# yannickBurkhardt/LongTermPlanner

Measured on AMD Instinct MI355X. Metric: 7-DoF trajectory plans/sec (batch 1M), higher is better.
Workload: dtype f64; 1 GPU; 1000000 x 7-DoF queries per GPU per step, limits 'panda', Tsample 0.001 s, full q/v/a/j sampling into a reused 192.0 GiB tile (2 chunks per step); batch_per_gpu=1000000, global_batch=1000000, dof=7, workload_key=panda:1000000:f64, limits=panda, input_layout=query_major, table_pass=auto, batches_in_flight=1, semantics=cpp, pow_rule=libm, backend=none (single rank), plans_ok_is=planTrajectory's bool

## Files before the change

### longtermplanner_amd/csrc/ltp_device.hpp

```cpp
#pragma once
#include "ltp_kernels.hpp"
#include "ltp_profile.hpp"

namespace ltp {

typedef double double2_t __attribute__((ext_vector_type(2)));
typedef float float4_t __attribute__((ext_vector_type(4)));

template <typename T> struct OutVec;
template <> struct OutVec<double> { typedef double2_t type; static constexpr int N = 2; };
template <> struct OutVec<float> { typedef float4_t type; static constexpr int N = 4; };

LTP_DEV LimPow load_limit_powers(const Limits& lim, int j)
{
    const double* w = lim.pw + (long long)j * kLimPowN;
    return LimPow{w[0], w[1], w[2], w[3], w[4], w[5], w[6]};
}

LTP_DEV JointLimits load_limits(const Limits& lim, int j)
{
    JointLimits L;
    L.q_min = lim.q_min[j];
    L.q_max = lim.q_max[j];
    L.v_max = lim.v_max[j];
    L.a_max = lim.a_max[j];
    L.j_max = lim.j_max[j];
    L.pw = load_limit_powers(lim, j);
    return L;
}

LTP_DEV int plan_set(const PlanLimits& lim, long long p)
{
    const int s = lim.set_index[p];
    return s >= 0 && s < lim.n_sets ? s : -1;
}

LTP_DEV Limits plan_limits(const PlanLimits& lim, long long p, int dof)
{
    if (!lim.set_index) return lim;
    const int s = plan_set(lim, p);
    const long long o = (long long)(s < 0 ? 0 : s) * dof, rows = lim.set_rows;
    return Limits{lim.sets + o, lim.sets + rows + o, lim.sets + 2 * rows + o, lim.sets + 3 * rows + o, lim.sets + 4 * rows + o,
                  lim.set_pw + o * kLimPowN};
}

struct PlanLane {
    bool live;
    long long local, p;
    int j;
    LTP_DEV void start(const Queries& in, double& q, double& v, double& a) const
    {
        const long long ix = p * in.sq + (long long)j * in.sj;
        q = in.q_0[ix];
        v = in.v_0[ix];
        a = in.a_0[ix];
    }
};
LTP_DEV PlanLane plan_lane(const PlanRange& r)
{
    const long long idx = (long long)blockIdx.x * blockDim.x + threadIdx.x;
    const long long local = idx / r.dof;
    return PlanLane{idx < r.count * r.dof, local, r.first + local, (int)(idx - local * r.dof)};
}

LTP_DEV bool beyond_end_limits(double q, double q_min, double q_max) { return q < q_min || q > q_max; }

LTP_DEV int joint_len(const double (&t)[7], double t_sample)
{
    bool finite = true;
#pragma unroll
    for (int k = 0; k < 7; ++k) finite = finite && dfinite(t[k]);
    const double len = dceil(t[6] / t_sample) + 1.0;
    return (finite && len < 2147483647.0) ? (int)len : -1;
}

LTP_HD int stored_len(int len, RowSpec rows)
{
    if (len <= 0) return 0;
    const int st = rows.stride > 1 ? rows.stride : 1;
    const int cnt = (len + st - 1) / st;
    return (rows.max_samples > 0 && cnt > rows.max_samples) ? rows.max_samples : cnt;
}

LTP_DEV unsigned long long plan_size(int len, int dof)
{
    if (len <= 0) return 0ull;
    const unsigned long long stride = ((unsigned long long)len + (kRowAlign - 1)) / kRowAlign * kRowAlign;
    return 4ull * (unsigned long long)dof * stride;
}

}
```

### longtermplanner_amd/csrc/ltp_sampler.hip

```cpp
#include "ltp_sampler_lds.hpp"

namespace ltp {

template <bool STREAMING, bool DRY, typename T>
__global__ void __launch_bounds__(kSampleThreads, (sizeof(T) == 4 ? kSampleBlocksPerCU - 1 : kSampleBlocksPerCU))
k_sample(long long first, long long count, int dof, double t_sample, PlanLimits lim, Queries in, Records rec,
         const unsigned long long* __restrict__ offsets, T* __restrict__ out, unsigned long long capacity,
         unsigned long long* __restrict__ stamps, int spread, RowSpec rows, unsigned long long* __restrict__ next_item,
         int draw_chunk )
{
    __shared__ SegTable tab;
    __shared__ unsigned long long s_item;
    const int ngroups = (dof + kSampleJointGroup - 1) / kSampleJointGroup;
    const long long per = (count + spread - 1) / spread;
    const unsigned long long total = (unsigned long long)per * spread * ngroups;
    const unsigned long long off0 = offsets[first];
    unsigned long long chunk_base = 0ull;
    int chunk_i = 0;
    auto draw = [&]() -> unsigned long long {
        if (chunk_i == 0) chunk_base = atomicAdd(next_item, (unsigned long long)draw_chunk);
        return chunk_base + (unsigned long long)chunk_i;
    };

    auto decode = [&](unsigned long long item, long long& local, int& j0, int& nj) {
        const int group = (int)(item % ngroups);
        const long long slot = (long long)(item / ngroups);
        local = (slot % spread) * per + slot / spread;
        j0 = group * kSampleJointGroup;
        nj = (dof - j0) < kSampleJointGroup ? (dof - j0) : kSampleJointGroup;
    };
    auto fetch = [&](unsigned long long item) {
        long long local; int j0, nj;
        decode(item, local, j0, nj);
        const bool some = item < total && local < count;
        return fetch_item<false>(some ? first + local : -1, j0, nj, dof, lim, in, rec, offsets);
    };

    if (threadIdx.x == 0) s_item = draw();
    chunk_i = (chunk_i + 1) & (draw_chunk - 1);
    __syncthreads();
    unsigned long long item = s_item;
    ItemRegs<false> cur = fetch(item);
    __syncthreads();
    while (item < total) {
        long long local; int j0, nj;
        decode(item, local, j0, nj);
        const long long p = first + local;
        const bool lead = threadIdx.x == 0 && j0 == 0;
        if (stamps && lead && local < count) stamps[3 * local] = wall_clock64();
        const int len = __builtin_amdgcn_readfirstlane(cur.len);
        const unsigned long long off = ((unsigned long long)(unsigned)__builtin_amdgcn_readfirstlane((int)(unsigned)(cur.off >> 32)) << 32) |
                                       (unsigned long long)(unsigned)__builtin_amdgcn_readfirstlane((int)(unsigned)cur.off);
        const unsigned long long rel = off - off0;
        const int slen = stored_len(len, rows);
        const unsigned long long stride = ((unsigned long long)slen + (kRowAlign - 1)) / kRowAlign * kRowAlign;
        bool ok = len > 0;
        if (ok && rel + 4ull * dof * stride > capacity) {
            if (lead) atomicOr(&rec.status[p], kStatusOverflow);
            ok = false;
        }
        unsigned long long drawn = 0ull;
        if (threadIdx.x == 0) drawn = draw();
        chunk_i = (chunk_i + 1) & (draw_chunk - 1);
        if (ok) build_run_tables(tab, p, j0, nj, len, t_sample, plan_limits(lim, p, dof), rec, cur.pa, cur.pb);
        if (threadIdx.x == 0) s_item = drawn;
        __syncthreads();
        const unsigned long long nitem = s_item;
        const ItemRegs<false> nxt = fetch(nitem);
        if (ok) {
            if (stamps && lead) stamps[3 * local + 1] = wall_clock64();
            stream_rows<STREAMING, DRY, T>(tab, j0, nj, dof, slen, stride, out + rel, rows);
        }
        __syncthreads();
        if (stamps && ok && lead) stamps[3 * local + 2] = wall_clock64();
        item = nitem;
        cur = nxt;
    }
}

int sample_resident_blocks(int device, bool f32)
{
    int cus = 0, per_cu = 0;
    if (hipDeviceGetAttribute(&cus, hipDeviceAttributeMultiprocessorCount, device) != hipSuccess || cus <= 0) cus = 256;
    hipError_t e;
    if (f32) e = hipOccupancyMaxActiveBlocksPerMultiprocessor(&per_cu, k_sample<true, false, float>, kSampleThreads, 0);
    else e = hipOccupancyMaxActiveBlocksPerMultiprocessor(&per_cu, k_sample<true, false, double>, kSampleThreads, 0);
    if (e != hipSuccess || per_cu <= 0) per_cu = 4;
    return cus * per_cu;
}

void launch_sample(hipStream_t s, const PlanRange& r, const unsigned long long* offsets, void* out, bool f32, unsigned long long capacity,
                   bool nontemporal, bool dry, int interleave, RowSpec rows, unsigned long long* next_item, int resident_blocks,
                   unsigned long long* stamps)
{
    const long long count = r.count;
    const int dof = r.dof;
    if (count <= 0) return;
    int spread = interleave != 0 ? interleave : kSampleSpread;
    if ((long long)spread > count) spread = (int)count;
    const int ngroups = (dof + kSampleJointGroup - 1) / kSampleJointGroup;
    long long blocks = resident_blocks > 0 ? resident_blocks : 1536;
    if (blocks > count * ngroups) blocks = count * ngroups;
    const dim3 grid((unsigned)blocks);
    const dim3 block(kSampleThreads);
    const int draw_chunk = queue_draw_chunk(rows, f32, dof < kSampleJointGroup ? dof : kSampleJointGroup);
#define LTP_SAMPLE_CASE(ST, DR, TY) hipLaunchKernelGGL((k_sample<ST, DR, TY>), grid, block, 0, s, r.first, count, dof, r.t_sample, r.lim, r.in, r.rec, offsets, (TY*)out, capacity, stamps, spread, rows, next_item, draw_chunk)
    switch ((nontemporal ? 1 : 0) | (dry ? 2 : 0) | (f32 ? 4 : 0)) {
    case 0: LTP_SAMPLE_CASE(false, false, double); break;
    case 1: LTP_SAMPLE_CASE(true, false, double); break;
    case 2: LTP_SAMPLE_CASE(false, true, double); break;
    case 3: LTP_SAMPLE_CASE(true, true, double); break;
    case 4: LTP_SAMPLE_CASE(false, false, float); break;
    case 5: LTP_SAMPLE_CASE(true, false, float); break;
    case 6: LTP_SAMPLE_CASE(false, true, float); break;
    default: LTP_SAMPLE_CASE(true, true, float); break;
    }
#undef LTP_SAMPLE_CASE
}

}
```

### longtermplanner_amd/csrc/ltp_sampler_lds.hpp

```cpp
#pragma once
#include "ltp_runs.hpp"

namespace ltp {

struct SegScratch {
    int s[kSampleJointGroup][8];
    double fr[kSampleJointGroup][8];
    double frts[kSampleJointGroup][8];
    double misc[kSampleJointGroup][8];
    double Jp[kSampleJointGroup][8];
    double corr[kSampleJointGroup][10];
    int cand[kSampleJointGroup][kMaxSegments];
    double runJ[kSampleJointGroup][kMaxSegments];
    int runMode[kSampleJointGroup][kMaxSegments];
    double state[kSampleJointGroup][kMaxSegments][3];
};
struct SegTable {
    JointTable jt[kSampleJointGroup];
    union {
        SegScratch w;
        double2_t bnd[kSampleJointGroup][kMaxSegments][4];
    };
};
static_assert(kSampleJointGroup == kRunTableJoints && kSampleThreads == kRunTableThreads, "install_run_tables is written for this block shape");

constexpr int kCutSlots = 20;
__device__ const signed char kCutBase[kCutSlots] = {0, 0, 0, 0, 1, 1, 2, 2, 2, 3, 3, 3, 4, 4, 4, 5, 5, 6, 6, 6};
__device__ const signed char kCutDelta[kCutSlots] = {0, 0, 1, 2, 0, 1, 0, 1, 2, -1, 0, 1, 0, 1, 2, 0, 1, 0, 1, 2};

LTP_DEV void wave_sync()
{
    __builtin_amdgcn_fence(__ATOMIC_RELEASE, "wavefront");
    __builtin_amdgcn_wave_barrier();
    __builtin_amdgcn_fence(__ATOMIC_ACQUIRE, "wavefront");
}

template <bool TABLES>
struct ItemRegs {
    int len;
    unsigned long long off;
    double pa, pb;
    unsigned long long w[kTableLoads];
};
template <>
struct ItemRegs<false> {
    int len;
    unsigned long long off;
    double pa, pb;
};

template <bool TABLES>
LTP_DEV ItemRegs<TABLES> fetch_item(long long p, int j0, int nj, int dof, const PlanLimits& lim, const Queries& in, const Records& rec,
                                    const unsigned long long* __restrict__ offsets,
                                    const unsigned long long* __restrict__ tables = nullptr, long long tab_first = 0)
{
    ItemRegs<TABLES> r;
    r.len = 0; r.off = 0ull; r.pa = 0.0; r.pb = 0.0;
    if constexpr (TABLES) {
#pragma unroll
        for (int x = 0; x < kTableLoads; ++x) r.w[x] = 0ull;
    }
    if (p < 0) return r;
    r.len = rec.traj_len[p];
    if (offsets) r.off = offsets[p];
    if constexpr (TABLES) {
        const PackedTableRegs t = fetch_run_tables(tables, (unsigned long long)(p - tab_first) * dof + j0, nj);
#pragma unroll
        for (int x = 0; x < kTableLoads; ++x) r.w[x] = t.w[x];
        return r;
    }
    const int jl = threadIdx.x >> 5, k = threadIdx.x & 31;
    if (jl < nj) {
        const int j = j0 + jl;
        const long long rj = p * dof + j;
        const long long ix = p * in.sq + (long long)j * in.sj;
        if (k < 7) r.pa = rec.t_scaled[rj * 7 + k];
        else if (k == 7) { r.pa = rec.dir[rj]; r.pb = plan_limits(lim, p, dof).j_max[j]; }
        else if (k == 8) { r.pa = rec.v_drive[rj]; r.pb = rec.dir[rj]; }
        else if (k == 9) r.pa = in.q_0[ix];
        else if (k == 10) r.pa = in.v_0[ix];
        else if (k == 11) r.pa = in.a_0[ix];
        else if (k == 12) r.pa = (double)rec.mod[rj];
    }
    return r;
}

template <bool PROBE = false>
LTP_DEV void build_run_tables(SegTable& tab, long long p, int j0, int nj, int len, double Ts, const Limits& lim,
                              const Records& rec, double pa, double pb, unsigned long long* probe = nullptr)
{
    __builtin_amdgcn_s_setprio(3);
    const int jl = threadIdx.x >> 5, k = threadIdx.x & 31;
    const bool jact = jl < nj;
    const int j = j0 + (jact ? jl : 0);
    if (jact && k < 7) {
        const double tk = pa;
        const double fr = tk - Ts * dfloor(tk / Ts);
        tab.w.fr[jl][k] = fr;
        tab.w.frts[jl][k] = fr / Ts;
        tab.w.s[jl][k] = (k & 1) ? (int)dceil(tk / Ts) : (int)dfloor(tk / Ts);
    } else if (jact && k < 13) {
        tab.w.misc[jl][k - 7] = k < 9 ? pa * pb : pa;
    }
    wave_sync();
    if constexpr (PROBE) { if (threadIdx.x == 0) probe[3] = wall_clock64(); }
    int cval = -1;
    if (jact && k == 8) {
        const double dj = tab.w.misc[jl][0];
        const bool modp = tab.w.misc[jl][5] == 1.0;
        const double J0 = dj * (modp ? -1.0 : 1.0), J2 = dj * (modp ? 1.0 : -1.0), J4 = dj * -1.0, J6 = dj * 1.0;
        tab.w.Jp[jl][0] = J0; tab.w.Jp[jl][1] = dj * 0.0; tab.w.Jp[jl][2] = J2; tab.w.Jp[jl][3] = dj * 0.0;
        tab.w.Jp[jl][4] = J4; tab.w.Jp[jl][5] = dj * 0.0; tab.w.Jp[jl][6] = J6;
        const double* ft = tab.w.frts[jl];
        const double d20 = (tab.w.fr[jl][2] - tab.w.fr[jl][0]) / Ts;
        tab.w.corr[jl][0] = ft[0] * J0;
        tab.w.corr[jl][1] = (1 - ft[1]) * J2;
        tab.w.corr[jl][2] = ft[2] * J2;
        tab.w.corr[jl][3] = d20 * J2;
        tab.w.corr[jl][4] = (1 - ft[3]) * J4;
        tab.w.corr[jl][5] = ft[4] * J4;
        tab.w.corr[jl][6] = 0.0;
        tab.w.corr[jl][7] = (1 - ft[5]) * J6;
        tab.w.corr[jl][8] = ft[6] * J6;
    }
    if (jact && k < kCutSlots) {
        const int c = k == 0 ? 0 : tab.w.s[jl][kCutBase[k]] + kCutDelta[k];
        cval = (k == 0 || (c > 0 && c < len)) ? c : -1;
        tab.w.cand[jl][k] = cval;
    }
    wave_sync();
    if constexpr (PROBE) { if (threadIdx.x == 0) probe[4] = wall_clock64(); }
    if (jact && k < kCutSlots) {
        bool first = cval >= 0;
#pragma unroll
        for (int m = 0; m < kCutSlots; ++m) first = first && (m >= k || tab.w.cand[jl][m] != cval);
        tab.w.runMode[jl][k] = first ? cval : -1;
    }
    wave_sync();
    if constexpr (PROBE) { if (threadIdx.x == 0) probe[5] = wall_clock64(); }
    if (jact && k < kCutSlots) {
        const bool mine = tab.w.runMode[jl][k] >= 0;
        int pos = 0, distinct = 0;
#pragma unroll
        for (int m = 0; m < kCutSlots; ++m) {
            const int cm = tab.w.runMode[jl][m];
            if (cm >= 0) { ++distinct; if (cm < cval) ++pos; }
        }
        if (mine) tab.jt[jl].start[pos] = cval;
        if (k == 0) { tab.jt[jl].start[distinct] = len; tab.jt[jl].nseg = distinct; }
    }
    wave_sync();
    if constexpr (PROBE) { if (threadIdx.x == 0) probe[6] = wall_clock64(); }
    const int ns = jact ? tab.jt[jl].nseg : 0;
    if (k < ns) {
        const int b = tab.jt[jl].start[k];
        const int* sj = tab.w.s[jl];
        const bool phase4 = sj[3] - sj[2] > 2;
        int mode = 0;
        if (b > sj[6]) mode |= kModeTail;
        if (phase4 && b >= sj[2] + 1 && b < sj[3] - 1) mode |= kModeVSnap;
        const double J = jerk_at(sj, tab.w.Jp[jl], tab.w.corr[jl], b);
        tab.w.runMode[jl][k] = mode;
        tab.w.runJ[jl][k] = J;
        reinterpret_cast<int*>(tab.jt[jl].c[k])[0] = tab.jt[jl].start[k + 1] - b;
    }
    wave_sync();
    if constexpr (PROBE) { if (threadIdx.x == 0) probe[7] = wall_clock64(); }
    if (jact && k == 0) {
        const double vsnap = tab.w.misc[jl][1];
        double q = tab.w.misc[jl][2], v = tab.w.misc[jl][3], a = tab.w.misc[jl][4];
        int mode = tab.w.runMode[jl][0], cnt = reinterpret_cast<const int*>(tab.jt[jl].c[0])[0];
        double J = tab.w.runJ[jl][0];
        for (int m = 0; m < ns; ++m) {
            const int mn = m + 1 < ns ? m + 1 : m;
            const int mode_n = tab.w.runMode[jl][mn], cnt_n = reinterpret_cast<const int*>(tab.jt[jl].c[mn])[0];
            const double J_n = tab.w.runJ[jl][mn];
            tab.w.state[jl][m][0] = a; tab.w.state[jl][m][1] = v; tab.w.state[jl][m][2] = q;
            const RunCoef rc = run_coef(mode, J, a, v, q, vsnap, Ts);
            double jj;
            run_eval(rc.c, cnt, q, v, a, jj);
            mode = mode_n; cnt = cnt_n; J = J_n;
        }
        if (beyond_end_limits(q, lim.q_min[j], lim.q_max[j])) atomicOr(&rec.status[p], kStatusEndLimit);
    }
    wave_sync();
    if constexpr (PROBE) { if (threadIdx.x == 0) probe[8] = wall_clock64(); }
    if (k < ns) {
        const RunCoef rc = run_coef(tab.w.runMode[jl][k], tab.w.runJ[jl][k], tab.w.state[jl][k][0], tab.w.state[jl][k][1],
                                    tab.w.state[jl][k][2], tab.w.misc[jl][1], Ts);
#pragma unroll
        for (int x = 0; x < kRunCoefs; ++x) tab.jt[jl].c[k][x] = rc.c[x];
    }
    __builtin_amdgcn_s_setprio(0);
}

template <bool STREAMING, bool DRY, typename T>
LTP_DEV void stream_rows(SegTable& tab, int j0, int nj, int dof, int slen, unsigned long long stride, T* __restrict__ plan_base,
                         RowSpec rows)
{
    typedef typename OutVec<T>::type V;
    constexpr int N = OutVec<T>::N;
    const unsigned long long arr_stride = (unsigned long long)dof * stride;
    const int nslots = (slen + N - 1) / N;
    const int sstride = rows.stride > 1 ? rows.stride : 1;

    if constexpr (!DRY) {
        const int jl = threadIdx.x >> 5, k = threadIdx.x & 31;
        const int nruns = jl < nj ? tab.jt[jl].nseg : 0;
        if (k < nruns) {
            const int* st = tab.jt[jl].start;
            const int u = k >= 1 ? (st[k] + sstride - 1) / sstride
                                 : slen;
            bool mine = (u % N) != 0 && u < N * nslots;
            if (mine && k > 1) {
                const int up = (st[k - 1] + sstride - 1) / sstride;
                if ((up % N) != 0 && up / N == u / N) mine = false;
            }
            if (mine) {
                const int i0 = u / N * N, t0 = i0 * sstride;
                int kh = k >= 1 ? k - 1 : nruns - 1;
                while (st[kh] > t0) --kh;
                int ch = st[kh], nh = kh + 1 < nruns ? st[kh + 1] : 0x7fffffff;
                V o[4];
#pragma unroll
                for (int h = 0; h < N; ++h) {
                    const int i = t0 + h * sstride;
                    while (nh <= i) {
                        ++kh;
                        ch = nh;
                        nh = kh + 1 < nruns ? st[kh + 1] : 0x7fffffff;
                    }
                    const bool pad = i0 + h >= slen;
                    double x4[4];
                    run_eval(tab.jt[jl].c[kh], i - ch + 1, x4[0], x4[1], x4[2], x4[3]);
#pragma unroll
                    for (int x = 0; x < 4; ++x) o[x][h] = pad ? (T)0 : (T)x4[x];
                }
#pragma unroll
                for (int x = 0; x < 4; ++x) *reinterpret_cast<V*>(&tab.bnd[jl][k][x]) = o[x];
            }
        }
        __syncthreads();
    }

    const int lw = nslots <= 64 ? 0 : (nslots <= 128 ? 1 : 2);
    const int wave = __builtin_amdgcn_readfirstlane((int)(threadIdx.x >> 6)), lane = threadIdx.x & 63;
    typedef unsigned int u32x4 __attribute__((ext_vector_type(4)));
    constexpr int kWindowSlots = 1 << 26;
    constexpr bool kBufferStores = STREAMING && sizeof(T) == 8;
    for (int jl2 = wave >> lw; jl2 < nj; jl2 += 4 >> lw) {
        T* const row = plan_base + (unsigned long long)(j0 + jl2) * stride;
        const int* st = tab.jt[jl2].start;
        const int nruns = tab.jt[jl2].nseg;
        int kr = 0, cur = 0, nxt = nruns > 1 ? st[1] : 0x7fffffff;
        for (int wbase = 0; wbase < nslots; wbase += kWindowSlots) {
            const int wend = nslots - wbase < kWindowSlots ? nslots : wbase + kWindowSlots;
            __amdgpu_buffer_rsrc_t rsrc[4];
            if constexpr (kBufferStores) {
#pragma unroll
                for (int x = 0; x < 4; ++x) {
                    rsrc[x] = __builtin_amdgcn_make_buffer_rsrc(row + x * arr_stride + (unsigned long long)wbase * N, 0,
                                                                (wend - wbase) * (int)sizeof(V), 0x00020000);
                }
            }
            for (int slot = wbase + ((wave & ((1 << lw) - 1)) << 6) + lane; slot < wend; slot += 64 << lw) {
                const int i0 = N * slot;
                V o[4];
                if constexpr (DRY) {
#pragma unroll
                    for (int x = 0; x < 4; ++x)
#pragma unroll
                        for (int h = 0; h < N; ++h) o[x][h] = (T)(i0 + h);
                } else {
                    const int t0 = i0 * sstride;
                    while (nxt <= t0) {
                        ++kr;
                        cur = nxt;
                        nxt = kr + 1 < nruns ? st[kr + 1] : 0x7fffffff;
                    }
                    const bool straddles = t0 + (N - 1) * sstride >= nxt;
                    if (straddles || i0 + N > slen) {
                        const int e = straddles ? kr + 1 : 0;
#pragma unroll
                        for (int x = 0; x < 4; ++x) o[x] = *reinterpret_cast<const V*>(&tab.bnd[jl2][e][x]);
                    } else {
                        double c[kRunCoefs];
#pragma unroll
                        for (int x = 0; x < kRunCoefs; ++x) c[x] = tab.jt[jl2].c[kr][x];
#pragma unroll
                        for (int h = 0; h < N; ++h) {
                            double x4[4];
                            run_eval(c, t0 + h * sstride - cur + 1, x4[0], x4[1], x4[2], x4[3]);
#pragma unroll
                            for (int x = 0; x < 4; ++x) o[x][h] = (T)x4[x];
                        }
                    }
                }
                if constexpr (kBufferStores) {
                    const unsigned voff = (unsigned)(slot - wbase) * (unsigned)sizeof(V);
#pragma unroll
                    for (int x = 0; x < 4; ++x)
                        __builtin_amdgcn_raw_buffer_store_b128(__builtin_bit_cast(u32x4, o[x]), rsrc[x], voff, 0,  2 | 16);
                } else if constexpr (STREAMING) {
#pragma unroll
                    for (int x = 0; x < 4; ++x) __builtin_nontemporal_store(o[x], reinterpret_cast<V*>(row + x * arr_stride + i0));
                } else {
#pragma unroll
                    for (int x = 0; x < 4; ++x) *reinterpret_cast<V*>(row + x * arr_stride + i0) = o[x];
                }
            }
        }
    }
}

}
```

Baseline: 17.86 million plans/s.

## Prefetch next item's plan words via scalar loads and deepen work-draw pipeline

The sampler kernel now draws work items two ahead, so the next item's index is known before the current one's tables are built. The next item's length, offset and limit set are loaded with scalar loads, and its per-lane operands are issued branch-free, all overlapping with the current table build. Lane shuffles then redistribute the j_max and mod values. The cut tables are packed into 64-bit constants instead of device-memory arrays. In exchange it adds an explicit vmcnt(0) wait before the barrier, more live registers, and more complex double-buffered item bookkeeping.

```diff
diff --git a/longtermplanner_amd/csrc/ltp_device.hpp b/longtermplanner_amd/csrc/ltp_device.hpp
--- a/longtermplanner_amd/csrc/ltp_device.hpp
+++ b/longtermplanner_amd/csrc/ltp_device.hpp
@@ -29,19 +29,20 @@
     return L;
 }
 
-LTP_DEV int plan_set(const PlanLimits& lim, long long p)
+LTP_DEV int checked_set(const PlanLimits& lim, int s) { return s >= 0 && s < lim.n_sets ? s : -1; }
+LTP_DEV int plan_set(const PlanLimits& lim, long long p) { return checked_set(lim, lim.set_index[p]); }
+
+LTP_DEV Limits set_limits(const PlanLimits& lim, int s, int dof)
 {
-    const int s = lim.set_index[p];
-    return s >= 0 && s < lim.n_sets ? s : -1;
+    if (!lim.set_index) return lim;
+    const long long o = (long long)(s < 0 ? 0 : s) * dof, rows = lim.set_rows;
+    return Limits{lim.sets + o, lim.sets + rows + o, lim.sets + 2 * rows + o, lim.sets + 3 * rows + o, lim.sets + 4 * rows + o,
+                  lim.set_pw + o * kLimPowN};
 }
-
 LTP_DEV Limits plan_limits(const PlanLimits& lim, long long p, int dof)
 {
     if (!lim.set_index) return lim;
-    const int s = plan_set(lim, p);
-    const long long o = (long long)(s < 0 ? 0 : s) * dof, rows = lim.set_rows;
-    return Limits{lim.sets + o, lim.sets + rows + o, lim.sets + 2 * rows + o, lim.sets + 3 * rows + o, lim.sets + 4 * rows + o,
-                  lim.set_pw + o * kLimPowN};
+    return set_limits(lim, plan_set(lim, p), dof);
 }
 
 struct PlanLane {
diff --git a/longtermplanner_amd/csrc/ltp_sampler.hip b/longtermplanner_amd/csrc/ltp_sampler.hip
--- a/longtermplanner_amd/csrc/ltp_sampler.hip
+++ b/longtermplanner_amd/csrc/ltp_sampler.hip
@@ -1,6 +1,10 @@
 #include "ltp_sampler_lds.hpp"
 
 namespace ltp {
+
+constexpr int kWaitVmcnt0 = 0x0F70;
+template <typename W>
+LTP_DEV W scalar_load(const W* p) { return *(const __attribute__((address_space(4))) W*)p; }
 
 template <bool STREAMING, bool DRY, typename T>
 __global__ void __launch_bounds__(kSampleThreads, (sizeof(T) == 4 ? kSampleBlocksPerCU - 1 : kSampleBlocksPerCU))
@@ -10,16 +14,22 @@
          int draw_chunk )
 {
     __shared__ SegTable tab;
-    __shared__ unsigned long long s_item;
+    __shared__ unsigned long long s_item[2], s_chunk;
     const int ngroups = (dof + kSampleJointGroup - 1) / kSampleJointGroup;
     const long long per = (count + spread - 1) / spread;
     const unsigned long long total = (unsigned long long)per * spread * ngroups;
     const unsigned long long off0 = offsets[first];
-    unsigned long long chunk_base = 0ull;
+    unsigned long long fresh = 0ull;
     int chunk_i = 0;
-    auto draw = [&]() -> unsigned long long {
-        if (chunk_i == 0) chunk_base = atomicAdd(next_item, (unsigned long long)draw_chunk);
-        return chunk_base + (unsigned long long)chunk_i;
+    auto draw = [&]() -> int {
+        const int place = chunk_i;
+        if (threadIdx.x == 0 && place == 0) fresh = atomicAdd(next_item, (unsigned long long)draw_chunk);
+        chunk_i = (place + 1) & (draw_chunk - 1);
+        return place;
+    };
+    auto take = [&](int place, unsigned long long& item) {
+        if (place == 0) s_chunk = fresh;
+        item = s_chunk + (unsigned long long)place;
     };
 
     auto decode = [&](unsigned long long item, long long& local, int& j0, int& nj) {
@@ -29,18 +39,35 @@
         j0 = group * kSampleJointGroup;
         nj = (dof - j0) < kSampleJointGroup ? (dof - j0) : kSampleJointGroup;
     };
-    auto fetch = [&](unsigned long long item) {
+    struct PlanWords {
+        int len;
+        unsigned long long off;
+        int set;
+    };
+    auto fetch = [&](unsigned long long item, PlanWords& w) {
         long long local; int j0, nj;
         decode(item, local, j0, nj);
         const bool some = item < total && local < count;
-        return fetch_item<false>(some ? first + local : -1, j0, nj, dof, lim, in, rec, offsets);
+        const long long pl = some ? first + local : -1;
+        w.len = some ? scalar_load(rec.traj_len + pl) : 0;
+        w.off = some ? scalar_load(offsets + pl) : 0ull;
+        w.set = some && lim.set_index ? checked_set(lim, scalar_load(lim.set_index + pl)) : -1;
+        return fetch_ahead(pl, j0, nj, dof, set_limits(lim, w.set, dof), in, rec);
+    };
+    auto uniform = [](unsigned long long v) {
+        return ((unsigned long long)(unsigned)__builtin_amdgcn_readfirstlane((int)(unsigned)(v >> 32)) << 32) |
+               (unsigned long long)(unsigned)__builtin_amdgcn_readfirstlane((int)(unsigned)v);
     };
 
-    if (threadIdx.x == 0) s_item = draw();
-    chunk_i = (chunk_i + 1) & (draw_chunk - 1);
+    const int place0 = draw();
+    if (threadIdx.x == 0) take(place0, s_item[0]);
+    const int place1 = draw();
+    if (threadIdx.x == 0) take(place1, s_item[1]);
     __syncthreads();
-    unsigned long long item = s_item;
-    ItemRegs<false> cur = fetch(item);
+    unsigned long long item = uniform(s_item[0]), nitem = uniform(s_item[1]);
+    PlanWords plan;
+    AheadRegs cur = fetch(item, plan);
+    __builtin_amdgcn_s_waitcnt(kWaitVmcnt0);
     __syncthreads();
     while (item < total) {
         long long local; int j0, nj;
@@ -48,10 +75,8 @@
         const long long p = first + local;
         const bool lead = threadIdx.x == 0 && j0 == 0;
         if (stamps && lead && local < count) stamps[3 * local] = wall_clock64();
-        const int len = __builtin_amdgcn_readfirstlane(cur.len);
-        const unsigned long long off = ((unsigned long long)(unsigned)__builtin_amdgcn_readfirstlane((int)(unsigned)(cur.off >> 32)) << 32) |
-                                       (unsigned long long)(unsigned)__builtin_amdgcn_readfirstlane((int)(unsigned)cur.off);
-        const unsigned long long rel = off - off0;
+        const int len = plan.len;
+        const unsigned long long rel = plan.off - off0;
         const int slen = stored_len(len, rows);
         const unsigned long long stride = ((unsigned long long)slen + (kRowAlign - 1)) / kRowAlign * kRowAlign;
         bool ok = len > 0;
@@ -59,14 +84,16 @@
             if (lead) atomicOr(&rec.status[p], kStatusOverflow);
             ok = false;
         }
-        unsigned long long drawn = 0ull;
-        if (threadIdx.x == 0) drawn = draw();
-        chunk_i = (chunk_i + 1) & (draw_chunk - 1);
-        if (ok) build_run_tables(tab, p, j0, nj, len, t_sample, plan_limits(lim, p, dof), rec, cur.pa, cur.pb);
-        if (threadIdx.x == 0) s_item = drawn;
+        const int place = draw();
+        PlanWords nplan;
+        double pa, pb;
+        finish_ahead(cur, pa, pb);
+        const AheadRegs nxt = fetch(nitem, nplan);
+        if (ok) build_run_tables(tab, p, j0, nj, len, t_sample, set_limits(lim, plan.set, dof), rec, pa, pb);
+        __builtin_amdgcn_s_waitcnt(kWaitVmcnt0);
+        if (threadIdx.x == 0) take(place, s_item[0]);
         __syncthreads();
-        const unsigned long long nitem = s_item;
-        const ItemRegs<false> nxt = fetch(nitem);
+        const unsigned long long nnitem = uniform(s_item[0]);
         if (ok) {
             if (stamps && lead) stamps[3 * local + 1] = wall_clock64();
             stream_rows<STREAMING, DRY, T>(tab, j0, nj, dof, slen, stride, out + rel, rows);
@@ -74,7 +101,9 @@
         __syncthreads();
         if (stamps && ok && lead) stamps[3 * local + 2] = wall_clock64();
         item = nitem;
+        nitem = nnitem;
         cur = nxt;
+        plan = nplan;
     }
 }
 
diff --git a/longtermplanner_amd/csrc/ltp_sampler_lds.hpp b/longtermplanner_amd/csrc/ltp_sampler_lds.hpp
--- a/longtermplanner_amd/csrc/ltp_sampler_lds.hpp
+++ b/longtermplanner_amd/csrc/ltp_sampler_lds.hpp
@@ -25,8 +25,17 @@
 static_assert(kSampleJointGroup == kRunTableJoints && kSampleThreads == kRunTableThreads, "install_run_tables is written for this block shape");
 
 constexpr int kCutSlots = 20;
-__device__ const signed char kCutBase[kCutSlots] = {0, 0, 0, 0, 1, 1, 2, 2, 2, 3, 3, 3, 4, 4, 4, 5, 5, 6, 6, 6};
-__device__ const signed char kCutDelta[kCutSlots] = {0, 0, 1, 2, 0, 1, 0, 1, 2, -1, 0, 1, 0, 1, 2, 0, 1, 0, 1, 2};
+constexpr signed char kCutBase[kCutSlots] = {0, 0, 0, 0, 1, 1, 2, 2, 2, 3, 3, 3, 4, 4, 4, 5, 5, 6, 6, 6};
+constexpr signed char kCutDelta[kCutSlots] = {0, 0, 1, 2, 0, 1, 0, 1, 2, -1, 0, 1, 0, 1, 2, 0, 1, 0, 1, 2};
+constexpr unsigned long long pack_cut_list(const signed char (&list)[kCutSlots], int bias)
+{
+    unsigned long long packed = 0ull;
+    for (int c = 0; c < kCutSlots; ++c) packed |= (unsigned long long)(list[c] + bias) << (3 * c);
+    return packed;
+}
+constexpr unsigned long long kCutBasePacked = pack_cut_list(kCutBase, 0), kCutDeltaPacked = pack_cut_list(kCutDelta, 1);
+LTP_DEV int cut_base(int c) { return (int)(kCutBasePacked >> (3 * c)) & 7; }
+LTP_DEV int cut_delta(int c) { return ((int)(kCutDeltaPacked >> (3 * c)) & 7) - 1; }
 
 LTP_DEV void wave_sync()
 {
@@ -83,6 +92,37 @@
         else if (k == 12) r.pa = (double)rec.mod[rj];
     }
     return r;
+}
+
+struct AheadRegs {
+    double w;
+    int mod;
+};
+LTP_DEV AheadRegs fetch_ahead(long long p, int j0, int nj, int dof, const Limits& lim , const Queries& in, const Records& rec)
+{
+    AheadRegs r;
+    r.w = 0.0; r.mod = 0;
+    if (p < 0) return r;
+    const int jl = threadIdx.x >> 5, k = threadIdx.x & 31;
+    const int j = j0 + (jl < nj ? jl : 0);
+    const long long rj = p * dof + j;
+    const long long ix = p * in.sq + (long long)j * in.sj;
+    const double* src = rec.dir + rj;
+    if (k < 7) src = rec.t_scaled + (rj * 7 + k);
+    else if (k == 8) src = rec.v_drive + rj;
+    else if (k == 9) src = in.q_0 + ix;
+    else if (k == 10) src = in.v_0 + ix;
+    else if (k == 11) src = in.a_0 + ix;
+    else if (k == 13) src = lim.j_max + j;
+    r.w = *src;
+    r.mod = rec.mod[rj];
+    return r;
+}
+LTP_DEV void finish_ahead(const AheadRegs& r, double& pa, double& pb)
+{
+    const int mod = __shfl_down(r.mod, 6, 32);
+    pb = __shfl_down(r.w, 6, 32);
+    pa = (threadIdx.x & 31) == 12 ? (double)mod : r.w;
 }
 
 template <bool PROBE = false>
@@ -124,7 +164,7 @@
         tab.w.corr[jl][8] = ft[6] * J6;
     }
     if (jact && k < kCutSlots) {
-        const int c = k == 0 ? 0 : tab.w.s[jl][kCutBase[k]] + kCutDelta[k];
+        const int c = k == 0 ? 0 : tab.w.s[jl][cut_base(k)] + cut_delta(k);
         cval = (k == 0 || (c > 0 && c < len)) ? c : -1;
         tab.w.cand[jl][k] = cval;
     }
```

Result: no change. 17.83 million plans/s (-0.2%).
